# nmichlo/mtg-vision

Hardware: AMD Instinct MI355X
Metric: cards/sec end-to-end (detect+embed+top-1 over 100k bank), 640x640 (higher is better)
Workload: dtype f32 (products as 3 x f16 MFMA on hi/lo-split operands, f32 accumulate)

## Files before the change

### include/mtgv.h

```cpp
#ifndef MTGV_H
#define MTGV_H

#include <stddef.h>
#include <stdint.h>

#ifdef __cplusplus
extern "C" {
#endif

#if defined(__GNUC__)
#define MTGV_API __attribute__((visibility("default")))
#else
#define MTGV_API
#endif

MTGV_API const char* mtgv_last_error(void);
MTGV_API int mtgv_version(void);
MTGV_API int mtgv_device_count(void);

#define MTGV_PREC_F32 0
#define MTGV_PREC_F16X3 1
MTGV_API int mtgv_set_gemm_precision(int32_t prec);
MTGV_API int mtgv_get_gemm_precision(int32_t* prec);

// ... 133 lines not shown
MTGV_API int mtgv_op_linear_ex(const float* a_dev, const float* w_dev, const float* bias_dev, const float* res_dev, float* out_dev,
                               int32_t m, int32_t n, int32_t k, int32_t act, int32_t hw, const float* a_scale_dev,
                               const float* a_shift_dev, float* grn_part_dev, void* stream);
MTGV_API int mtgv_op_conv2d(const float* x_dev, const float* w_dev, const float* bias_dev, float* out_dev, int32_t n, int32_t h,
                            int32_t w, int32_t cin, int32_t cout, int32_t kh, int32_t kw, int32_t stride, int32_t pad,
                            int32_t act, void* stream);
MTGV_API int mtgv_op_layernorm(const float* x_dev, const float* w_dev, const float* b_dev, float* out_dev, int64_t rows,
                               int32_t c, float eps, void* stream);
MTGV_API int mtgv_op_dwconv7(const float* x_dev, const float* w49_dev, const float* bias_dev, float* out_dev, int32_t n,
                             int32_t h, int32_t w, int32_t c, void* stream);
MTGV_API int mtgv_op_block(const float* x_dev, float* out_dev, int32_t n, int32_t h, int32_t w, int32_t c, int32_t act,
                           const float* dw_w49, const float* dw_b, const float* ln_w, const float* ln_b, const float* w1,
                           const float* b1, const float* gamma, const float* beta, const float* w2, const float* b2,
                           float* ws_dev, void* stream);
MTGV_API int64_t mtgv_op_block_workspace_floats(int32_t n, int32_t h, int32_t w, int32_t c);
MTGV_API int mtgv_op_l2norm(const float* x_dev, float* out_dev, int64_t rows, int32_t d, void* stream);

#ifdef __cplusplus
}
#endif
#endif
```

### mtg-vision_amd/csrc/api.hip

```cpp
#include "mtgv.h"

#include <math.h>
#include <string.h>
#include <algorithm>
#include <mutex>

#include "encoder.h"
#include "match.h"
#include "rowops.h"
#include "gemm_sp.h"

namespace mtgv {
const char* last_error_cstr();
}

using namespace mtgv;

namespace {
std::recursive_mutex g_op_mu;
struct ScopedWeights {
  const float* w = nullptr;
  hipStream_t s;
  std::unique_lock<std::recursive_mutex> lk;
  ScopedWeights(const float* W, int n, int k, hipStream_t stream) : s(stream), lk(g_op_mu) {
// ... 305 lines not shown
    bw.dw_w49 = (float*)dw_w49, bw.dw_b = (float*)dw_b, bw.ln_w = (float*)ln_w, bw.ln_b = (float*)ln_b;
    bw.w1 = (float*)w1, bw.b1 = (float*)b1, bw.gamma = (float*)gamma, bw.beta = (float*)beta;
    bw.w2 = (float*)w2, bw.b2 = (float*)b2;
    ScopedWeights reg1(w1, 4 * c, c, (hipStream_t)stream), reg2(w2, c, 4 * c, (hipStream_t)stream);
    const BlockWsSize z = block_ws_size(n, h, w, c);
    BlockWs ws;
    ws.t1 = ws_dev;
    ws.t2 = ws.t1 + z.t;
    ws.hid = ws.t2 + z.t;
    ws.part = ws.hid + z.hid;
    ws.scale = ws.part + z.part;
    ws.bfold = ws.scale + z.scale;
    run_block(x_dev, out_dev, n, h, w, c, act, bw, ws, (hipStream_t)stream);
  });
}
MTGV_API int mtgv_op_l2norm(const float* x_dev, float* out_dev, int64_t rows, int32_t d, void* stream) {
  return guarded([&] {
    MTGV_CHECK(x_dev && out_dev, ERR_INVALID, "null argument");
    l2norm_rows_launch(x_dev, out_dev, rows, d, (hipStream_t)stream);
  });
}

}
```

### mtg-vision_amd/csrc/encoder.hip

```cpp
#include "encoder.h"
#include <stdlib.h>
#include "rowops.h"
#include "gemm_sp.h"
#include "mlp_fused.h"

#include <string.h>

namespace mtgv {

void DevBuf::alloc(size_t floats) {
  release();
  if (floats == 0) return;
  HIP_OK(hipMalloc((void**)&p, floats * sizeof(float)));
  n = floats;
}
void DevBuf::release() {
  if (p) (void)hipFree(p);
  p = nullptr;
  n = 0;
}

ParamStore::~ParamStore() {
  for (auto& kv : slots_)
    if (kv.second.dev) {
// ... 119 lines not shown
      fold_shift_into_bias_launch(bw.w2, bw.beta, bw.b2, ws.bfold, c, 4 * c, s);
      m.b2 = ws.bfold;
    }
    if (ln != nullptr && ln->out_sp8 != nullptr) m.out_ln = ln->out_sp8, m.ln_w = ln->w, m.ln_b = ln->b, m.ln_eps = ln->eps;
    mlp_fused_launch(m, s);
    return m.out_ln != nullptr;
  }

  GemmArgs g1 = linear_args(ws.t2, c, bw.w1, bw.b1, ws.hid, 4 * c, M, 4 * c, c, act);
  g1.a_fmt = fmt;
  g1.hw = hw;
  g1.grn_part = ws.part;
  const GrnLayout gl = gemm_grn_layout(g1);
  gemm_launch(g1, s);

  grn_finalize_launch(ws.part, gl, n, hw, 4 * c, bw.gamma, ws.scale, s);

  GemmArgs g2 = linear_args(ws.hid, 4 * c, bw.w2, bw.b2, out, c, M, c, 4 * c, ACT_NONE);
  g2.res = x;
  g2.ldr = c;
  g2.hw = hw;
  g2.a_scale = ws.scale;
  if (bw.b2_folded != nullptr) {
    g2.bias = bw.b2_folded;
  } else {
    fold_shift_into_bias_launch(bw.w2, bw.beta, bw.b2, ws.bfold, c, 4 * c, s);
    g2.bias = ws.bfold;
  }
  gemm_launch(g2, s);
  return false;
}

static std::string blk_key(int kind, int s, int j, const char* leaf) {
  char b[128];
  if (kind == MTGV_ENC_AE)
    snprintf(b, sizeof(b), "block%d.2.%d.%s", s, j, leaf);
  else
// ... 221 lines not shown
  MTGV_CHECK(x != nullptr && z_out != nullptr, ERR_INVALID, "null tensor");
  if (!prepared_) prepare();
  const int H = cfg_.image_h, W = cfg_.image_w;
  const float sc = cfg_.scale_io ? 2.0f : 1.0f, sf = cfg_.scale_io ? -1.0f : 0.0f;
  if (layout == MTGV_IN_NCHW_F32)
    nchw_to_nhwc_launch((const float*)x, x0_.p, n, 3, H, W, 3, sc, sf, s);
  else if (layout == MTGV_IN_NHWC_F32)
    f32hwc_scale_launch((const float*)x, x0_.p, (long)n * H * W, 3, 3, sc, sf, s);
  else if (layout == MTGV_IN_NHWC_U8)
    u8_to_f32_launch((const uint8_t*)x, x0_.p, (long)n * H * W, 3, 3, sc, sf, 0, s);
  else
    MTGV_CHECK(false, ERR_INVALID, "unknown input layout %d", layout);

  if (graph_mode_ != 0 && !capture_ && n <= graph_max_n_ && !gemm_profile_enabled()) {
    zbuf_.ensure((size_t)cfg_.max_batch * cfg_.z_size);
    const int gkey = n * 2 + gemm_precision();
    auto it = graphs_.find(gkey);
    if (it == graphs_.end()) {
      body(n, zbuf_.p, s);
      hipGraph_t graph = nullptr;
      hipGraphExec_t exec = nullptr;
      if (cap_stream_ == nullptr) HIP_OK(hipStreamCreateWithFlags(&cap_stream_, hipStreamNonBlocking));
      HIP_OK(hipStreamBeginCapture(cap_stream_, hipStreamCaptureModeThreadLocal));
      try {
        body(n, zbuf_.p, cap_stream_);
      } catch (...) {
        (void)hipStreamEndCapture(cap_stream_, &graph);
        if (graph) (void)hipGraphDestroy(graph);
        throw;
      }
      HIP_OK(hipStreamEndCapture(cap_stream_, &graph));
// ... 118 lines not shown
```

### mtg-vision_amd/csrc/gemm_f32.h

```cpp
#pragma once
#include "common.h"

namespace mtgv {

struct GemmArgs {
  const float* A = nullptr;
  int a_fmt = 0;
  const float* W = nullptr;
  const float* W_split = nullptr;
  const float* wscale = nullptr;
  float a_mul = 1.0f, a_unmul = 1.0f;
  float* Out = nullptr;
  int out_fmt = 0;
  const float* bias = nullptr;
  const float* res = nullptr;
  int res_fmt = 0;
  int M = 0, N = 0, K = 0;

  int H = 1, Wd = 1;
  int c_total = 0;
  int c_off = 0;
  int Cin = 0;
  int KH = 1, KW = 1, stride = 1, pad = 0;
  int stride_w = 0;
// ... 3 lines not shown
  int os = 1, oy = 0, ox = 0, OH2 = 1, OW2 = 1;
  int os_nq = 0;
  const float* W2 = nullptr;
  const float* bias2 = nullptr;
  float* Out2 = nullptr;
  int N2 = 0, ldo2 = 0, o_off2 = 0, out_fmt2 = 0, act2 = ACT_NONE;
  int ldr = 0;
  int act = ACT_NONE;

  float* grn_part = nullptr;
  int hw = 0;
  int segmax = 0;
  int grn_unit_rows = 0;
  const float* a_scale = nullptr;
  const float* a_shift = nullptr;

  int batch = 1;
  long strideA = 0, strideW = 0, strideO = 0;
  const int* m_count = nullptr;
  const float* crop_boxes = nullptr;
  int crop_rows = 0;
  float crop_scale = 0.f;
  int crop_w = 1;

  float* cand_s = nullptr;
  int* cand_i = nullptr;
  int topk = 0;
  const float* ln_w = nullptr;
  const float* ln_b = nullptr;
  float ln_eps = 0.f;
// ... 19 lines not shown
void gemm_profile_enable(bool on);
bool gemm_profile_enabled();
void gemm_profile_read(double* ms, double* flops, long* launches);
void gemm_profile_dump(const char* path);
double gemm_profile_bytes();
void gemm_profile_begin(const GemmArgs& a, hipStream_t s, int sp, double fill, double bytes);
void gemm_profile_end(hipStream_t s);

struct GrnLayout {
  int unit_rows = 0, segmax = 0;
  size_t floats = 0;
};
GrnLayout gemm_grn_layout(const GemmArgs& a);
size_t gemm_grn_part_floats_max(int M, int N, int hw);

void grn_finalize_launch(const float* part, const GrnLayout& l, int n_img, int hw, int N, const float* gamma, float* scale,
                         hipStream_t s);

}
```

### mtg-vision_amd/csrc/gemm_f32.hip

```cpp
#include "gemm_kernel.h"
#include "gemm_sp.h"

#include <stdlib.h>
#include <string.h>
#include <algorithm>
#include <map>
#include <mutex>
#include <string>
#include <vector>

namespace mtgv {

bool gemm_dispatch_f32(const GemmDev& g, const GemmPlan& pl, bool conv, bool apro, int grid, hipStream_t s) {
  return gemm_dispatch<0>(g, pl, conv, apro, grid, s);
}
bool gemm_dispatch_f16x3(const GemmDev& g, const GemmPlan& pl, bool conv, bool apro, int grid, hipStream_t s);


namespace {
struct GemmProf {
  bool on = false;
  std::vector<hipEvent_t> ev;
  size_t used = 0;
  double flops = 0;
// ... 34 lines not shown
double gemm_profile_bytes() { return g_prof.bytes; }

void gemm_profile_read(double* ms, double* flops, long* launches) {
  double total = 0;
  for (size_t i = 0; i + 1 < g_prof.used; i += 2) {
    HIP_OK(hipEventSynchronize(g_prof.ev[i + 1]));
    float t = 0.f;
    HIP_OK(hipEventElapsedTime(&t, g_prof.ev[i], g_prof.ev[i + 1]));
    total += t;
  }
  if (ms) *ms = total;
  if (flops) *flops = g_prof.flops;
  if (launches) *launches = g_prof.launches;
}

static void prof_begin(const GemmArgs& a, const GemmPlan& pl, hipStream_t s, int sp, double fill, double bytes_override = -1.0) {
  if (!g_prof.on) return;
  while (g_prof.ev.size() < g_prof.used + 2) {
    hipEvent_t e;
    HIP_OK(hipEventCreate(&e));
    g_prof.ev.push_back(e);
  }
  HIP_OK(hipEventRecord(g_prof.ev[g_prof.used], s));
  const double xfl = a.W2 != nullptr ? 2.0 * (double)a.M * a.N2 * a.N : 0.0;
  g_prof.flops += 2.0 * (double)a.M * a.N * a.K * a.batch + xfl;
  {
    const double a_el = is_conv(a) ? (double)(a.M / (a.OH * a.OW)) * a.H * a.Wd * a.Cin : (double)a.M * a.K;
    const double w_el = (double)a.N * a.K;
    const double o_el = a.topk > 0 ? (double)a.M * ceil_div(a.N, 64) * a.topk * 2
                                   : (a.W2 != nullptr ? (double)a.M * a.N2 + (double)a.N2 * a.N : (double)a.M * a.N);
    const double r_el = a.res != nullptr ? (double)a.M * a.N : 0.0;
    double by = 4.0 * ((a.strideA != 0 || a.batch == 1 ? a.batch : 1) * a_el + (a.strideW != 0 || a.batch == 1 ? a.batch : 1) * w_el +
                       a.batch * (o_el + r_el));
    if (bytes_override >= 0.0) by = bytes_override;
    g_prof.bytes += by;
    g_prof.recs.push_back({a.M, a.N, a.K, a.KH, a.stride, a.batch, a.act, a.a_scale != nullptr, a.grn_part != nullptr, a.topk,
                           pl.tm, pl.tn, pl.bk, sp, by, fill, xfl});
  }
  g_prof.launches += 1;
}
static void prof_end(hipStream_t s) {
  if (!g_prof.on) return;
  HIP_OK(hipEventRecord(g_prof.ev[g_prof.used + 1], s));
  g_prof.used += 2;
}

__global__ __launch_bounds__(256) void split_pack_kernel(const float* __restrict__ in, float* __restrict__ out, long n4) {
  const long i = (long)blockIdx.x * 256 + threadIdx.x;
  if (i >= n4) return;
// ... 210 lines not shown
  MTGV_CHECK((long)a.M * (long)(a.OH * a.OW > a.hw ? a.OH * a.OW : a.hw) < (1l << 40), ERR_INVALID, "gemm: M too large for fastdiv");
  const bool conv = is_conv(a);
  const bool apro = a.a_scale != nullptr;
  MTGV_CHECK(!(apro && conv), ERR_INVALID, "gemm: GRN prologue only on 1x1");
  MTGV_CHECK(!(apro && a.act != ACT_NONE), ERR_INVALID, "gemm: GRN prologue is only combined with a linear epilogue");
  MTGV_CHECK(a.a_shift == nullptr, ERR_INVALID, "gemm: fold the GRN shift into the bias (fold_shift_into_bias_launch)");
  if (!conv) MTGV_CHECK(a.OH == a.H && a.OW == a.Wd, ERR_INVALID, "gemm: 1x1 geometry mismatch");
  if (apro || a.grn_part) MTGV_CHECK(a.hw > 0 && a.M % a.hw == 0, ERR_INVALID, "gemm: hw=%d must divide M=%d", a.hw, a.M);
  const SpPlan sp = gemm_sp_plan(a);
  if (a.grn_part) {
    const GrnLayout l = grn_layout(a, sp, pl);
    a.segmax = l.segmax;
    a.grn_unit_rows = l.unit_rows;
  }
  if (sp.cfg >= 0) {
    prof_begin(a, pl, s, 1, g_prof.on ? gemm_sp_fill_bytes(a, sp) : 0.0);
    gemm_sp_launch(a, sp, s);
    prof_end(s);
    return;
  }

  MTGV_CHECK(a.os_nq == 0, ERR_INVALID, "gemm: the grouped scatter epilogue (os_nq) exists on the LDS-DMA kernel only");
  MTGV_CHECK(a.W2 == nullptr, ERR_INVALID, "gemm: the chained 1x1 exists on the LDS-DMA kernel only");
  GemmDev g;
  g.a = a;
  if (gemm_precision() == GEMM_PREC_F16X3 && g.a.W_split == nullptr && a.strideW == 0)
    g.a.W_split = split_for_launch(a.W, a.K, &g.a.wscale);
  if (gemm_precision() != GEMM_PREC_F16X3) g.a.W_split = nullptr, g.a.wscale = nullptr;
  g.d_ohw = make_fastdiv((uint32_t)(a.OH * a.OW));
  g.d_ow = make_fastdiv((uint32_t)a.OW);
  g.d_cin = make_fastdiv((uint32_t)a.Cin);
// ... 52 lines not shown
    }
    const float gval = sqrtf(sum);
    gx[n] = gval;
    local += gval;
  }
  red[tid] = local;
  __syncthreads();
  for (int st = 128; st > 0; st >>= 1) {
    if (tid < st) red[tid] += red[tid + st];
    __syncthreads();
  }
  const float denom = red[0] / (float)N + 1e-6f;
  for (int n = tid; n < N; n += 256) scale[(long)img * N + n] = gamma[n] * (gx[n] / denom) + 1.0f;
}

__global__ __launch_bounds__(256) void fold_shift_kernel(const float* __restrict__ W, const float* __restrict__ shift,
                                                        const float* __restrict__ bias, float* __restrict__ out, int N, int K) {
  const int lane = threadIdx.x & 63;
  const int n = blockIdx.x * 4 + (threadIdx.x >> 6);
  if (n >= N) return;
  float acc = 0.f;
  for (int k = lane; k < K; k += 64) acc += W[(long)n * K + k] * shift[k];
#pragma unroll
  for (int m = 32; m > 0; m >>= 1) acc += __shfl_xor(acc, m);
  if (lane == 0) out[n] = acc + (bias != nullptr ? bias[n] : 0.f);
}

void fold_shift_into_bias_launch(const float* W, const float* shift, const float* bias, float* out, int N, int K, hipStream_t s) {
  hipLaunchKernelGGL(fold_shift_kernel, dim3((N + 3) / 4), dim3(256), 0, s, W, shift, bias, out, N, K);
  HIP_OK(hipGetLastError());
}

void grn_finalize_launch(const float* part, const GrnLayout& l, int n_img, int hw, int N, const float* gamma, float* scale,
                         hipStream_t s) {
  const size_t lds = (size_t)(N + 256) * sizeof(float);
  MTGV_CHECK(lds <= 160 * 1024, ERR_INVALID, "grn_finalize: N=%d too large", N);
  hipLaunchKernelGGL(grn_finalize_kernel, dim3(n_img), dim3(256), lds, s, part, l.unit_rows, l.segmax, hw, N,
                     make_fastdiv((uint32_t)hw), make_fastdiv((uint32_t)l.unit_rows), gamma, scale);
  HIP_OK(hipGetLastError());
}

}
```

### mtg-vision_amd/csrc/gemm_sp.h

```cpp
#pragma once
#include "gemm_f32.h"

namespace mtgv {

void sp8_register(const float* W, size_t n_floats, int row_k);
void sp8_refresh(const float* W, size_t offset_floats, size_t n_floats, hipStream_t s);
void sp8_unregister(const float* W);
bool sp8_lookup(const float* W, int K, const char** sp8, const float** wscale);

struct SpPlan {
  int cfg = -1;
  int bm = 0, bn = 0;
  int unit_rows = 0;
  int tiles_m = 0, tiles_n = 0;
};

bool gemm_sp_active();
SpPlan gemm_sp_plan(const GemmArgs& a);
bool gemm_sp_takes_sp8(const float* W, int M, int N, int K, int lda, int c_off);
void gemm_sp_launch(const GemmArgs& a, const SpPlan& pl, hipStream_t s);
bool gemm_sp_chain_ok(const GemmArgs& a);
bool gemm_sp_topk_layout(const GemmArgs& a, int* slots, int* cols);
double gemm_sp_fill_bytes(const GemmArgs& a, const SpPlan& pl);
void gemm_sp_stamps_dump(const char* path);

void gemm_sp_topk_hi16_launch(const void* q_hi, const void* bank_hi, const float* wscale, int b, int N, int K, int kp, float* cand_s,
                              int* cand_i, int* slots, hipStream_t s);
int gemm_sp_topk_hi16_slots(int N);
int gemm_sp_topk_hi16_range_cols();

const char* sp_zero_page();

void sp8_pack_plain_launch(const float* in, void* out, long rows, int K, hipStream_t s);

}
```

### mtg-vision_amd/csrc/gemm_sp.hip

```cpp
#include "gemm_sp.h"

#include <stdlib.h>
#include <map>
#include <mutex>
#include <vector>

#include "gemm_sp_kernel.h"

namespace mtgv {

__global__ __launch_bounds__(256) void sp8_pack_rows_kernel(const float* __restrict__ in, sp_h8* __restrict__ out,
                                                           float* __restrict__ wscale, long rows, int K) {
  const int lane = threadIdx.x & 63;
  const long row = (long)blockIdx.x * 4 + (threadIdx.x >> 6);
  if (row >= rows) return;
  const float* x = in + row * K;
  float mx = 0.f;
  for (int k = lane; k < K; k += 64) mx = fmaxf(mx, fabsf(x[k]));
#pragma unroll
  for (int m = 32; m > 0; m >>= 1) mx = fmaxf(mx, __shfl_xor(mx, m));
  int e = 0;
  if (mx > 0.f && mx < INFINITY) {
    int ex;
    (void)frexpf(mx, &ex);
// ... 266 lines not shown
bool stamps_on() {
  static const bool on = [] { const char* e = getenv("MTGV_SP_STAMPS"); return e != nullptr && atoi(e) != 0; }();
  return on;
}
}

bool gemm_sp_topk_layout(const GemmArgs& a, int* slots, int* cols) {
  const SpPlan pl = gemm_sp_plan(a);
  if (pl.cfg < 0) return false;
  const SpCfg& k = kCfg[pl.cfg];
  *slots = pl.tiles_n * k.wn;
  *cols = 32 * k.tn;
  return true;
}

double gemm_sp_fill_bytes(const GemmArgs& a, const SpPlan& pl) {
  const SpCfg& k = kCfg[pl.cfg];
  const double tiles = (double)pl.tiles_m * pl.tiles_n;
  const double b_tile = (double)k.bn() * a.K * 4.0;
  double a_tile = (double)k.bm() * a.K * 4.0;
  if (a.a_fmt == 1 && is_conv(a) && window_conv_fits(a, pl)) a_tile = (double)window_bytes(k, a.Wd) * (a.Cin / k.kps());
  if (a.a_scale != nullptr) a_tile += (double)(a.K / 32) * 1024.0;
  return tiles * (a_tile + b_tile);
}

void gemm_sp_stamps_dump(const char* path) {
  if (g_stamps.empty()) return;
  HIP_OK(hipDeviceSynchronize());
  FILE* f = fopen(path, "wb");
  MTGV_CHECK(f != nullptr, ERR_RUNTIME, "cannot open %s", path);
  std::vector<long> host;
  for (const StampRec& r : g_stamps) {
    const int hdr[8] = {r.M, r.N, r.K, r.cfg, r.amode, r.act, r.tiles, 0};
    fwrite(hdr, sizeof(int), 8, f);
    host.resize((size_t)r.tiles * 8);
    HIP_OK(hipMemcpy(host.data(), r.buf, host.size() * sizeof(long), hipMemcpyDeviceToHost));
    fwrite(host.data(), sizeof(long), host.size(), f);
// ... 76 lines not shown
    g.W2 = w28, g.wscale2 = w2s, g.bias2 = a.bias2, g.Out2 = a.Out2, g.ldo2 = a.ldo2, g.o_off2 = a.o_off2, g.out_fmt2 = a.out_fmt2;
    g.act2 = a.act2, g.N2 = a.N2;
  }
  g.nq = a.os_nq;
  g.d_nq = make_fastdiv((uint32_t)(a.os_nq > 0 ? a.os_nq : 1)), g.d_os = make_fastdiv((uint32_t)(a.os > 0 ? a.os : 1));
  if (a.os_nq > 0)
    MTGV_CHECK(g.remap && a.os_nq % 8 == 0 && a.N == a.os * a.os * a.os_nq && a.oy == 0 && a.ox == 0 && a.res == nullptr &&
                   a.grn_part == nullptr,
               ERR_INVALID, "gemm_sp: os_nq=%d does not describe a %dx%d scatter of N=%d columns", a.os_nq, a.os, a.os, a.N);
  int amode = a.a_fmt == 1 ? (is_conv(a) ? 2 : 0) : 1;
  if (amode == 2 && window_conv_fits(a, pl)) amode = 5;
  if (amode == 1 && g.a_mul == 1.0f && ((uintptr_t)g.A & 15) == 0) {
    if (g.a_scale == nullptr) amode = 4;
    else if (((uintptr_t)g.a_scale & 15) == 0 && (kCfg[pl.cfg].bm() - 1) / g.hw + 2 <= 8) amode = 3;
  }
  if (stamps_on() && gemm_profile_enabled()) {
    const int tiles = pl.tiles_m * pl.tiles_n;
    long* buf = nullptr;
    HIP_OK(hipMalloc(&buf, (size_t)tiles * 8 * sizeof(long)));
    HIP_OK(hipMemsetAsync(buf, 0, (size_t)tiles * 8 * sizeof(long), s));
    g.stamps = buf;
    g_stamps.push_back({a.M, a.N, a.K, pl.cfg, amode, a.act, tiles, buf});
  }
  switch (pl.cfg) {
    case 0: gemm_sp_launch_cfg0(g, amode, s); break;
    case 1: gemm_sp_launch_cfg1(g, amode, s); break;
    case 2: gemm_sp_launch_cfg2(g, amode, s); break;
    case 3: gemm_sp_launch_cfg3(g, amode, s); break;
    case 4: gemm_sp_launch_cfg4(g, amode, s); break;
    case 5: gemm_sp_launch_cfg5(g, amode, s); break;
// ... 8 lines not shown
```

### mtg-vision_amd/csrc/gemm_sp_inst.h

```cpp
#pragma once
#include "gemm_sp_kernel.h"

namespace mtgv {

namespace {
#ifndef SP_KS_VALUE
#define SP_KS_VALUE 2
#endif
constexpr int SP_KS = SP_KS_VALUE;
#ifndef SP_NST
#define SP_NST 2
#endif

template <int AMODE, int ACT, int EPI, int NST = SP_NST>
void sp_launch_nst(const SpDev& g, hipStream_t s) {
  constexpr int BM = 32 * SP_TM * SP_WM, BN = 32 * SP_TN * SP_WN;
  constexpr size_t ring = (size_t)NST * ((AMODE == 5 ? BN : BM + BN) * 64 * SP_KS + (AMODE == 3 ? 1024 : 0));
  size_t lds = ring;
  constexpr size_t chain_lds = (size_t)SP_WM * SP_WN * 4096 * (1 + SP_TN) + (size_t)SP_TN * 96 * 128;
  if (AMODE == 5) {
    constexpr int RB = 64 * SP_KS, RPP = 1024 / RB;
    const size_t win = (size_t)((BM + 2 * g.Wd + 2 + RPP - 1) / RPP * RPP) * RB;
    const size_t stage = (size_t)SP_WM * SP_WN * 32 * 128 * SP_TN;
    lds = win + ring > stage ? win + ring : stage;
  }
  if (EPI == 32 && lds < chain_lds) lds = chain_lds;
  static bool attr_done_dev[MTGV_MAX_DEVICES] = {};
  bool& attr_done = attr_done_dev[current_device()];
  auto kern = gemm_sp_kernel<SP_WM, SP_WN, SP_TM, SP_TN, SP_KS, NST, AMODE, ACT, EPI>;
  if (!attr_done) {
    HIP_OK(hipFuncSetAttribute((const void*)kern, hipFuncAttributeMaxDynamicSharedMemorySize, (AMODE == 5 || EPI == 32) ? 160 * 1024 : (int)lds));
    attr_done = true;
  }
  hipLaunchKernelGGL(kern, dim3((unsigned)(g.tiles_m * g.tiles_n)), dim3(64 * SP_WM * SP_WN), lds, s, g);
}

template <int AMODE, int ACT, int EPI>
void sp_launch_one(const SpDev& g, hipStream_t s) {
  if constexpr (AMODE == 5 && SP_NST == 2) {
    constexpr int BM = 32 * SP_TM * SP_WM, BN = 32 * SP_TN * SP_WN, RB = 64 * SP_KS, RPP = 1024 / RB;
    const size_t win = (size_t)((BM + 2 * g.Wd + 2 + RPP - 1) / RPP * RPP) * RB;
    if ((long)g.tiles_m * g.tiles_n <= 512 && win + (size_t)4 * BN * RB <= 80 * 1024) {
      sp_launch_nst<AMODE, ACT, EPI, 4>(g, s);
      return;
    }
  }
// ... 54 lines not shown
      case ACT_MISH: sp_pick<0, ACT_MISH, 8>(g, epi, s); break;
      case ACT_GELU: sp_pick<0, ACT_GELU, 8>(g, epi, s); break;
      case ACT_SILU: sp_pick<0, ACT_SILU, 1, 5>(g, epi, s); break;
      default: sp_pick<0, -1>(g, epi, s); break;
    }
  } else if (amode == 1) {
#if SP_NST == 2
    if (g.act == ACT_NONE) sp_pick<1, ACT_NONE>(g, epi, s);
    else sp_pick<1, -1>(g, epi, s);
#else
    MTGV_CHECK(false, ERR_RUNTIME, "gemm_sp: the register A path has no deep-ring instance");
#endif
  } else if (amode == 3) {
    if (g.act == ACT_NONE) sp_pick<3, ACT_NONE, 2>(g, epi, s);
    else sp_pick<3, -1>(g, epi, s);
  } else if (amode == 4) {
    if (g.act == ACT_NONE) sp_pick<4, ACT_NONE, 0, 2>(g, epi, s);
    else sp_pick<4, -1>(g, epi, s);
  } else if (amode == 5) {
#if SP_NST == 2
    switch (g.act) {
#if SP_WN == 1 && SP_TM == 1
      case ACT_SILU: sp_pick<5, ACT_SILU, 1, 5, 32>(g, epi, s); break;
#else
      case ACT_SILU: sp_pick<5, ACT_SILU, 1, 5>(g, epi, s); break;
#endif
      default: sp_pick<5, -1>(g, epi, s); break;
    }
#else
    MTGV_CHECK(false, ERR_RUNTIME, "gemm_sp: the window conv has no deep-ring instance");
// ... 17 lines not shown
```

### mtg-vision_amd/csrc/gemm_sp_kernel.h

```cpp
#pragma once
#include <type_traits>

#include "act.h"
#include "gemm_f32.h"
#include "sp8.h"

namespace mtgv {

typedef float spf16 __attribute__((ext_vector_type(16)));

__device__ __forceinline__ spf16 sp_mfma(sp_h8 b, sp_h8 a, spf16 c) {
  return __builtin_amdgcn_mfma_f32_32x32x16_f16(b, a, c, 0, 0, 0);
}

struct SpDev {
  float* cand_s = nullptr;
  int* cand_i = nullptr;
  int topk = 0;
  long* stamps = nullptr;
  const char* A = nullptr;
  long a_rowb = 0;
  long a_offb = 0;
  const char* W = nullptr;
  const float* wscale = nullptr;
  const float* bias = nullptr;
  const void* res = nullptr;
  long ldr = 0;
  int res_fmt = 0;
  float* Out = nullptr;
  long ldo = 0;
  int o_off = 0;
  int out_fmt = 0;
  int M = 0, N = 0, K = 0;
  float* grn_part = nullptr;
  int hw = 1, segmax = 0;
  FastDiv d_hw;
  const float* a_scale = nullptr;
  float a_mul = 1.0f, a_unmul = 1.0f;
  const char* zero = nullptr;
  int off32 = 0;
  int tiles_m = 0, tiles_n = 0;
  int act = 0;
  int H = 1, Wd = 1, Cin = 0, KW = 1, stride = 1, pad = 0, OH = 1, OW = 1;
  FastDiv d_ohw, d_ow, d_cin, d_kw;
  int remap = 0, os = 1, oy = 0, ox = 0, OH2 = 1, OW2 = 1;
  int nq = 0;
  FastDiv d_nq, d_os;
  const char* W2 = nullptr;
  const float* wscale2 = nullptr;
  const float* bias2 = nullptr;
  float* Out2 = nullptr;
  long ldo2 = 0;
// ... 1 lines not shown
};

typedef const __attribute__((address_space(1))) void* sp_gptr;
typedef __attribute__((address_space(3))) void* sp_lptr;

template <int WM, int WN, int TM, int TN, int KS, int NST, int AMODE, int ACT, int EPI>
__global__ __launch_bounds__(64 * WM * WN, (WM * WN == 8 ? 4 : 2)) void gemm_sp_kernel(const SpDev g) {
#pragma clang fp contract(off)
  constexpr int NW = WM * WN, NT = 64 * NW, BM = 32 * TM * WM, BN = 32 * TN * WN;
  constexpr bool GEN = EPI < 0;
  static_assert(TM <= 2, "the epilogue names its slabs");
  static_assert(NST >= 2 && NST <= 4 && (AMODE != 1 || NST == 2), "ring depth; the register A path is two-deep");
  constexpr int RB = 64 * KS, RPP = 1024 / RB, SPR = RB / 16;
  constexpr bool AWIN = AMODE == 5;
  constexpr bool ADMA = AMODE != 1 && !AWIN;
  constexpr bool AF32 = AMODE == 3 || AMODE == 4;
  constexpr bool HI16 = AMODE == 6;
  constexpr int EB = HI16 ? 2 : 4;
  static_assert(!HI16 || (KS == 2 && EPI == 16), "fp16 rows: 128-byte stage rows, top-k epilogue");
  constexpr int SA = AWIN ? 0 : BM * RB, SB = BN * RB, SSC = AMODE == 3 ? 1024 : 0, STG = SA + SB + SSC;
  static_assert(AMODE != 3 || KS == 2, "the scale image is one DMA piece: 8 images x 32 k");
  constexpr int PA = ADMA ? BM / RPP : 0, PB = BN / RPP, NP = PA + PB;
  constexpr int PPW = (NP + NW - 1) / NW;
  constexpr int CPS = BM * 2 * KS;
  constexpr int CPT = AMODE == 1 ? CPS / NT : 1;
  static_assert(AMODE != 1 || CPS % NT == 0, "A chunks must divide over the threads");
  extern __shared__ __attribute__((aligned(1024))) char smem[];

  const int tid = threadIdx.x, lane = tid & 63;
  const int wave = __builtin_amdgcn_readfirstlane(tid >> 6);
  const int wm = wave / WN, wn = wave % WN;
// ... 46 lines not shown
        const uint32_t ow = rem - oh * (uint32_t)g.OW;
        cih0[u] = (int)oh * g.stride - g.pad;
        ciw0[u] = (int)ow * g.stride - g.pad;
        csrc[u] = g.A + (((long)img * g.H + cih0[u]) * g.Wd + ciw0[u]) * g.a_rowb + g.a_offb + slot * 16;
        src[u] = g.A + (long)img * g.H * g.Wd * g.a_rowb + g.a_offb + (slot & 1) * 16;
      } else {
        src[u] = g.A + (long)m * g.a_rowb + g.a_offb + slot * 16;
      }
    } else {
      int n = n0 + row;
      n = n < g.N ? n : g.N - 1;
      src[u] = g.W + (long)n * wrowb + slot * 16;
    }
    tailz[u] = ktail && ((nk - 1) * 2 * KS + (slot >> 1)) >= kchunks;
  }
  const int img0 = AMODE == 3 ? (int)fdiv((uint32_t)m0, g.d_hw) : 0;
  const char* sc_src = nullptr;
  bool sc_tailz = false;
  if constexpr (AMODE == 3) {
    const int img_last = (int)fdiv((uint32_t)(g.M - 1), g.d_hw);
    const int im = img0 + (lane >> 3) < img_last ? img0 + (lane >> 3) : img_last;
    sc_src = reinterpret_cast<const char*>(g.a_scale + (long)im * g.K) + (lane & 7) * 16;
    sc_tailz = ktail && ((nk - 1) * 2 * KS + ((lane & 7) >> 1)) >= kchunks;
  }
  const int win_px = AWIN ? ((BM + 2 * g.Wd + 2 + RPP - 1) / RPP * RPP) : 0;
  char* const ring = smem + (AWIN ? win_px * RB : 0);
  auto issue_piece = [&](int u, int t, int buf) {
    const int p = wave + NW * u;
    const char* s;
    if (AMODE == 2 && p < PA && conv_fast) {
      const uint32_t k0 = (uint32_t)t * (16u * KS);
// ... 147 lines not shown
  const int swr = KS == 2 ? (r >> 1) & 7 : (r >> 2) & 3;
  unsigned a_off[TM], b_off[TN];
#pragma unroll
  for (int i = 0; i < TM; ++i) a_off[i] = (unsigned)((wm * TM * 32 + i * 32 + r) * RB);
#pragma unroll
  for (int j = 0; j < TN; ++j) b_off[j] = (unsigned)(SA + (wn * TN * 32 + j * 32 + r) * RB);
  unsigned sc_off[TM];
#pragma unroll
  for (int i = 0; i < TM; ++i) {
    sc_off[i] = 0;
    if constexpr (AMODE == 3) {
      int m = m0 + wm * TM * 32 + i * 32 + r;
      m = m < g.M ? m : g.M - 1;
      sc_off[i] = (unsigned)(SA + SB + ((int)fdiv((uint32_t)m, g.d_hw) - img0) * 128 + h * 32);
    }
  }

  const int nw0 = n0 + wn * TN * 32;
  const int mw0 = m0 + wm * TM * 32;
  const int slot = lane & 7, lrow = lane >> 3;
  sp_f4 wsc[TN], bsv[TN];
  bool col_ok[TN];
  auto load_colvecs = [&]() {
#pragma unroll
  for (int j = 0; j < TN; ++j) {
    const int n = nw0 + j * 32 + slot * 4;
    col_ok[j] = n < g.N;
    sp_f4 w1 = {1.f, 1.f, 1.f, 1.f}, b0 = {0.f, 0.f, 0.f, 0.f};
    if (n + 4 <= g.N) {
      if (g.wscale != nullptr) w1 = *reinterpret_cast<const sp_f4*>(g.wscale + n);
      if (g.bias != nullptr) b0 = *reinterpret_cast<const sp_f4*>(g.bias + n);
    } else if (GEN && n < g.N) {
#pragma unroll
      for (int e = 0; e < 4; ++e)
        if (n + e < g.N) {
          if (g.wscale != nullptr) w1[e] = g.wscale[n + e];
          if (g.bias != nullptr) b0[e] = g.bias[n + e];
        }
    }
    wsc[j] = w1 * g.a_unmul;
    bsv[j] = b0;
  }
  };
  load_colvecs();

  const bool wave_active = m0 + wm * TM * 32 < g.M;

  int my_pieces = 0;
#pragma unroll
  for (int u = 0; u < PPW; ++u) my_pieces += (NP % NW == 0 || wave + NW * u < NP) ? 1 : 0;
  if (AMODE == 3 && wave == NP % NW) my_pieces += 1;
  constexpr int AHEAD = NST - 2;
  auto wait_stage = [&](bool tail) {
    if (AHEAD == 0 || tail) {
      asm volatile("s_waitcnt vmcnt(0) lgkmcnt(0)" ::: "memory");
    } else if (my_pieces == PPW) {
      asm volatile("s_waitcnt vmcnt(%0) lgkmcnt(0)" ::"n"(PPW * AHEAD) : "memory");
    } else if (my_pieces == PPW + 1) {
      asm volatile("s_waitcnt vmcnt(%0) lgkmcnt(0)" ::"n"((PPW + 1) * AHEAD) : "memory");
// ... 90 lines not shown
          sp_h8 ah[TM], bh[TN];
  #pragma unroll
          for (int i = 0; i < TM; ++i) ah[i] = *reinterpret_cast<const sp_h8*>(sb + a_off[i] + so);
  #pragma unroll
          for (int j = 0; j < TN; ++j) bh[j] = *reinterpret_cast<const sp_h8*>(sb + b_off[j] + so);
  #pragma unroll
          for (int j = 0; j < TN; ++j)
  #pragma unroll
            for (int i = 0; i < TM; ++i) acc[i][j] = sp_mfma(bh[j], ah[i], acc[i][j]);
        }
      }
      if constexpr (AF32 && KS == 2 && !HI16) {
        __builtin_amdgcn_sched_barrier(0);
        if (wave_active) {
          const char* const sb = ring + buf * STG;
          sp_f4 xa[2][TM][2], xs[2][TM][2];
          sp_h8 bh[2][TN], bl[2][TN];
  #pragma unroll
          for (int ks = 0; ks < 2; ++ks) {
            const unsigned shi = (unsigned)(((ks * 4 + h * 2 + 0) ^ swr) << 4);
            const unsigned slo = (unsigned)(((ks * 4 + h * 2 + 1) ^ swr) << 4);
  #pragma unroll
            for (int i = 0; i < TM; ++i) {
              xa[ks][i][0] = *reinterpret_cast<const sp_f4*>(sb + a_off[i] + shi);
              xa[ks][i][1] = *reinterpret_cast<const sp_f4*>(sb + a_off[i] + slo);
              if constexpr (AMODE == 3) {
                xs[ks][i][0] = *reinterpret_cast<const sp_f4*>(sb + sc_off[i] + ks * 64);
                xs[ks][i][1] = *reinterpret_cast<const sp_f4*>(sb + sc_off[i] + ks * 64 + 16);
              }
            }
  #pragma unroll
            for (int j = 0; j < TN; ++j) {
              bh[ks][j] = *reinterpret_cast<const sp_h8*>(sb + b_off[j] + shi);
              bl[ks][j] = *reinterpret_cast<const sp_h8*>(sb + b_off[j] + slo);
            }
          }
          if constexpr (AMODE == 3) {
  #pragma unroll
            for (int ks = 0; ks < 2; ++ks)
  #pragma unroll
              for (int i = 0; i < TM; ++i) xa[ks][i][0] = xa[ks][i][0] * xs[ks][i][0], xa[ks][i][1] = xa[ks][i][1] * xs[ks][i][1];
          }
          sp_h8 ah[2][TM], al[2][TM];
  #pragma unroll
          for (int i = 0; i < TM; ++i) sp8_split8_mix(xa[0][i][0], xa[0][i][1], ah[0][i], al[0][i]);
  #pragma unroll
          for (int ks = 0; ks < 2; ++ks) {
            if (ks == 0) {
  #pragma unroll
              for (int i = 0; i < TM; ++i) sp8_split8_mix(xa[1][i][0], xa[1][i][1], ah[1][i], al[1][i]);
            }
  #pragma unroll
            for (int j = 0; j < TN; ++j)
  #pragma unroll
              for (int i = 0; i < TM; ++i) acc[i][j] = sp_mfma(bl[ks][j], ah[ks][i], acc[i][j]);
  #pragma unroll
            for (int j = 0; j < TN; ++j)
  #pragma unroll
              for (int i = 0; i < TM; ++i) acc[i][j] = sp_mfma(bh[ks][j], al[ks][i], acc[i][j]);
  #pragma unroll
            for (int j = 0; j < TN; ++j)
  #pragma unroll
              for (int i = 0; i < TM; ++i) acc[i][j] = sp_mfma(bh[ks][j], ah[ks][i], acc[i][j]);
          }
          constexpr int CV = (AMODE == 3 ? 8 : 0) + 16;
          __builtin_amdgcn_sched_group_barrier(0x100, 2 * (TM * (AMODE == 3 ? 4 : 2) + 2 * TN), 0);
          __builtin_amdgcn_sched_group_barrier(0x002, CV * TM, 0);
  #pragma unroll
          for (int q = 0; q < 3 * TM * TN; ++q) {
            __builtin_amdgcn_sched_group_barrier(0x008, 1, 0);
            __builtin_amdgcn_sched_group_barrier(0x002, (CV * TM + 3 * TM * TN - 1) / (3 * TM * TN), 0);
          }
        }
      } else if (wave_active && !HI16) {
        const char* const sb = ring + buf * STG;
  #pragma unroll
        for (int ks = 0; ks < KS; ++ks) {
          const unsigned shi = (unsigned)(((ks * 4 + h * 2 + 0) ^ swr) << 4);
          const unsigned slo = (unsigned)(((ks * 4 + h * 2 + 1) ^ swr) << 4);
          sp_h8 ah[TM], al[TM], bh[TN], bl[TN];
  #pragma unroll
// ... 405 lines not shown
```

### mtg-vision_amd/mtgv/native.py

```python

from __future__ import annotations

import ctypes as C
import os

import torch

_HERE = os.path.dirname(os.path.abspath(__file__))
LIB_PATH = os.environ.get("MTGV_LIB_PATH", os.path.join(_HERE, "libmtgv.so"))

c_i32, c_i64, c_f32, c_vp = C.c_int32, C.c_int64, C.c_float, C.c_void_p
c_fp = C.POINTER(C.c_float)


class EncoderCfg(C.Structure):
    _fields_ = [
        ("kind", c_i32),
        ("image_h", c_i32),
        ("image_w", c_i32),
        ("in_chans", c_i32),
        ("z_size", c_i32),
        ("depths", c_i32 * 4),
        ("dims", c_i32 * 4),
        ("head_type", c_i32),
# ... 74 lines not shown
    "mtgv_jpeg_decode": (C.c_int, [c_vp, c_vp, c_vp, c_vp, c_i32, c_vp, c_vp, c_vp, c_vp, c_vp]),
    "mtgv_jpeg_encode_bound": (C.c_int, [c_i32, c_i32, c_i32, C.POINTER(c_i64)]),
    "mtgv_jpeg_encode_header": (C.c_int, [c_i32, c_i32, c_i32, c_i32, c_vp, c_i64, C.POINTER(c_i64)]),
    "mtgv_jpeg_encoder_create": (C.c_int, [c_i32, c_i64, C.POINTER(c_vp)]),
    "mtgv_jpeg_encoder_destroy": (None, [c_vp]),
    "mtgv_jpeg_encode": (C.c_int, [c_vp, c_vp, c_i32, c_i32, c_i32, c_i32, c_i32, c_vp, c_i64, c_vp, c_vp]),
    "mtgv_op_linear": (C.c_int, [c_vp, c_vp, c_vp, c_vp, c_vp, c_i32, c_i32, c_i32, c_i32, c_vp]),
    "mtgv_op_linear_ex_part_floats": (c_i64, [c_i32, c_i32, c_i32, c_i32, c_i32]),
    "mtgv_op_last_grn_layout": (C.c_int, [c_vp, c_vp]),
    "mtgv_op_linear_ex": (C.c_int, [c_vp, c_vp, c_vp, c_vp, c_vp, c_i32, c_i32, c_i32, c_i32, c_i32, c_vp, c_vp, c_vp, c_vp]),
    "mtgv_op_conv2d": (C.c_int, [c_vp, c_vp, c_vp, c_vp] + [c_i32] * 10 + [c_vp]),
    "mtgv_op_layernorm": (C.c_int, [c_vp, c_vp, c_vp, c_vp, c_i64, c_i32, c_f32, c_vp]),
    "mtgv_op_dwconv7": (C.c_int, [c_vp, c_vp, c_vp, c_vp, c_i32, c_i32, c_i32, c_i32, c_vp]),
    "mtgv_op_block": (C.c_int, [c_vp, c_vp, c_i32, c_i32, c_i32, c_i32, c_i32] + [c_vp] * 10 + [c_vp, c_vp]),
    "mtgv_op_block_workspace_floats": (c_i64, [c_i32, c_i32, c_i32, c_i32]),
    "mtgv_op_l2norm": (C.c_int, [c_vp, c_vp, c_i64, c_i32, c_vp]),
}

_lib = None


def lib():
    global _lib
    if _lib is None:
        if not os.path.exists(LIB_PATH):
            raise RuntimeError(
                f"{LIB_PATH} is missing: build it with `python mtg-vision_amd/build.py` "
                "(mtgv has no CPU or eager fallback for the recognition path)"
            )
        L = C.CDLL(LIB_PATH)
# ... 49 lines not shown
```

Baseline: 32730.

## Derive GRN scale inside the second MLP GEMM prologue instead of a finalize kernel

Adds a new A-mode (7) to the split-precision GEMM kernel. In this mode each workgroup reduces the GRN partial sums for the images its tile touches, computes the per-channel scale table in LDS, and applies it while loading A. The separate grn_finalize kernel launch between the two MLP GEMMs is skipped whenever the inline path qualifies. The trade-off is that every tile redundantly re-reads and reduces the partials and uses extra LDS, which may reduce occupancy. An env var toggle, launch counters and a graph key bit are added.

```diff
diff --git a/include/mtgv.h b/include/mtgv.h
--- a/include/mtgv.h
+++ b/include/mtgv.h
@@ -171,6 +171,7 @@
                            const float* b1, const float* gamma, const float* beta, const float* w2, const float* b2,
                            float* ws_dev, void* stream);
 MTGV_API int64_t mtgv_op_block_workspace_floats(int32_t n, int32_t h, int32_t w, int32_t c);
+MTGV_API int mtgv_grn_launch_counts(int64_t* finalize, int64_t* inline_derived);
 MTGV_API int mtgv_op_l2norm(const float* x_dev, float* out_dev, int64_t rows, int32_t d, void* stream);
 
 #ifdef __cplusplus
diff --git a/mtg-vision_amd/csrc/api.hip b/mtg-vision_amd/csrc/api.hip
--- a/mtg-vision_amd/csrc/api.hip
+++ b/mtg-vision_amd/csrc/api.hip
@@ -343,6 +343,14 @@
     run_block(x_dev, out_dev, n, h, w, c, act, bw, ws, (hipStream_t)stream);
   });
 }
+MTGV_API int mtgv_grn_launch_counts(int64_t* finalize, int64_t* inline_derived) {
+  return guarded([&] {
+    MTGV_CHECK(finalize && inline_derived, ERR_INVALID, "null argument");
+    long f = 0, d = 0;
+    gemm_grn_launch_counts(&f, &d);
+    *finalize = f, *inline_derived = d;
+  });
+}
 MTGV_API int mtgv_op_l2norm(const float* x_dev, float* out_dev, int64_t rows, int32_t d, void* stream) {
   return guarded([&] {
     MTGV_CHECK(x_dev && out_dev, ERR_INVALID, "null argument");
diff --git a/mtg-vision_amd/csrc/encoder.hip b/mtg-vision_amd/csrc/encoder.hip
--- a/mtg-vision_amd/csrc/encoder.hip
+++ b/mtg-vision_amd/csrc/encoder.hip
@@ -157,13 +157,13 @@
   const GrnLayout gl = gemm_grn_layout(g1);
   gemm_launch(g1, s);
 
-  grn_finalize_launch(ws.part, gl, n, hw, 4 * c, bw.gamma, ws.scale, s);
-
   GemmArgs g2 = linear_args(ws.hid, 4 * c, bw.w2, bw.b2, out, c, M, c, 4 * c, ACT_NONE);
   g2.res = x;
   g2.ldr = c;
   g2.hw = hw;
   g2.a_scale = ws.scale;
+  g2.grn_src = ws.part, g2.grn_src_unit_rows = gl.unit_rows, g2.grn_src_segmax = gl.segmax, g2.grn_gamma = bw.gamma;
+  if (!gemm_derives_grn(g2)) grn_finalize_launch(ws.part, gl, n, hw, 4 * c, bw.gamma, ws.scale, s);
   if (bw.b2_folded != nullptr) {
     g2.bias = bw.b2_folded;
   } else {
@@ -415,7 +415,7 @@
 
   if (graph_mode_ != 0 && !capture_ && n <= graph_max_n_ && !gemm_profile_enabled()) {
     zbuf_.ensure((size_t)cfg_.max_batch * cfg_.z_size);
-    const int gkey = n * 2 + gemm_precision();
+    const int gkey = (n * 2 + gemm_precision()) * 2 + (gemm_grn_inline_enabled() ? 1 : 0);
     auto it = graphs_.find(gkey);
     if (it == graphs_.end()) {
       body(n, zbuf_.p, s);
diff --git a/mtg-vision_amd/csrc/gemm_f32.h b/mtg-vision_amd/csrc/gemm_f32.h
--- a/mtg-vision_amd/csrc/gemm_f32.h
+++ b/mtg-vision_amd/csrc/gemm_f32.h
@@ -41,6 +41,9 @@
   int grn_unit_rows = 0;
   const float* a_scale = nullptr;
   const float* a_shift = nullptr;
+  const float* grn_src = nullptr;
+  int grn_src_unit_rows = 0, grn_src_segmax = 0;
+  const float* grn_gamma = nullptr;
 
   int batch = 1;
   long strideA = 0, strideW = 0, strideO = 0;
@@ -90,6 +93,10 @@
 GrnLayout gemm_grn_layout(const GemmArgs& a);
 size_t gemm_grn_part_floats_max(int M, int N, int hw);
 
+bool gemm_derives_grn(const GemmArgs& a);
+bool gemm_grn_inline_enabled();
+void gemm_grn_launch_counts(long* finalize, long* inline_derived);
+
 void grn_finalize_launch(const float* part, const GrnLayout& l, int n_img, int hw, int N, const float* gamma, float* scale,
                          hipStream_t s);
 
diff --git a/mtg-vision_amd/csrc/gemm_f32.hip b/mtg-vision_amd/csrc/gemm_f32.hip
--- a/mtg-vision_amd/csrc/gemm_f32.hip
+++ b/mtg-vision_amd/csrc/gemm_f32.hip
@@ -4,6 +4,7 @@
 #include <stdlib.h>
 #include <string.h>
 #include <algorithm>
+#include <atomic>
 #include <map>
 #include <mutex>
 #include <string>
@@ -72,7 +73,8 @@
   if (launches) *launches = g_prof.launches;
 }
 
-static void prof_begin(const GemmArgs& a, const GemmPlan& pl, hipStream_t s, int sp, double fill, double bytes_override = -1.0) {
+static void prof_begin(const GemmArgs& a, const GemmPlan& pl, hipStream_t s, int sp, double fill, double bytes_override = -1.0,
+                       double bytes_extra = 0.0) {
   if (!g_prof.on) return;
   while (g_prof.ev.size() < g_prof.used + 2) {
     hipEvent_t e;
@@ -91,6 +93,7 @@
     double by = 4.0 * ((a.strideA != 0 || a.batch == 1 ? a.batch : 1) * a_el + (a.strideW != 0 || a.batch == 1 ? a.batch : 1) * w_el +
                        a.batch * (o_el + r_el));
     if (bytes_override >= 0.0) by = bytes_override;
+    by += bytes_extra;
     g_prof.bytes += by;
     g_prof.recs.push_back({a.M, a.N, a.K, a.KH, a.stride, a.batch, a.act, a.a_scale != nullptr, a.grn_part != nullptr, a.topk,
                            pl.tm, pl.tn, pl.bk, sp, by, fill, xfl});
@@ -331,7 +334,9 @@
     a.grn_unit_rows = l.unit_rows;
   }
   if (sp.cfg >= 0) {
-    prof_begin(a, pl, s, 1, g_prof.on ? gemm_sp_fill_bytes(a, sp) : 0.0);
+    const bool derives = g_prof.on && gemm_sp_derives_grn(a, sp);
+    prof_begin(a, pl, s, 1, g_prof.on ? gemm_sp_fill_bytes(a, sp) : 0.0, -1.0,
+               derives ? (double)ceil_div(a.M, a.grn_src_unit_rows) * a.grn_src_segmax * a.K * 4.0 : 0.0);
     gemm_sp_launch(a, sp, s);
     prof_end(s);
     return;
@@ -414,6 +419,13 @@
   for (int n = tid; n < N; n += 256) scale[(long)img * N + n] = gamma[n] * (gx[n] / denom) + 1.0f;
 }
 
+static std::atomic<long> g_grn_finalize_launches{0};
+void gemm_grn_inline_count(long* n);
+void gemm_grn_launch_counts(long* finalize, long* inline_derived) {
+  *finalize = g_grn_finalize_launches.load();
+  gemm_grn_inline_count(inline_derived);
+}
+
 __global__ __launch_bounds__(256) void fold_shift_kernel(const float* __restrict__ W, const float* __restrict__ shift,
                                                         const float* __restrict__ bias, float* __restrict__ out, int N, int K) {
   const int lane = threadIdx.x & 63;
@@ -433,6 +445,7 @@
 
 void grn_finalize_launch(const float* part, const GrnLayout& l, int n_img, int hw, int N, const float* gamma, float* scale,
                          hipStream_t s) {
+  g_grn_finalize_launches += 1;
   const size_t lds = (size_t)(N + 256) * sizeof(float);
   MTGV_CHECK(lds <= 160 * 1024, ERR_INVALID, "grn_finalize: N=%d too large", N);
   hipLaunchKernelGGL(grn_finalize_kernel, dim3(n_img), dim3(256), lds, s, part, l.unit_rows, l.segmax, hw, N,
diff --git a/mtg-vision_amd/csrc/gemm_sp.h b/mtg-vision_amd/csrc/gemm_sp.h
--- a/mtg-vision_amd/csrc/gemm_sp.h
+++ b/mtg-vision_amd/csrc/gemm_sp.h
@@ -21,6 +21,7 @@
 void gemm_sp_launch(const GemmArgs& a, const SpPlan& pl, hipStream_t s);
 bool gemm_sp_chain_ok(const GemmArgs& a);
 bool gemm_sp_topk_layout(const GemmArgs& a, int* slots, int* cols);
+bool gemm_sp_derives_grn(const GemmArgs& a, const SpPlan& pl);
 double gemm_sp_fill_bytes(const GemmArgs& a, const SpPlan& pl);
 void gemm_sp_stamps_dump(const char* path);
 
diff --git a/mtg-vision_amd/csrc/gemm_sp.hip b/mtg-vision_amd/csrc/gemm_sp.hip
--- a/mtg-vision_amd/csrc/gemm_sp.hip
+++ b/mtg-vision_amd/csrc/gemm_sp.hip
@@ -1,6 +1,7 @@
 #include "gemm_sp.h"
 
 #include <stdlib.h>
+#include <atomic>
 #include <map>
 #include <mutex>
 #include <vector>
@@ -304,13 +305,47 @@
   return true;
 }
 
+namespace {
+std::atomic<long> g_grn_inline_launches{0};
+int grn_units_per_image(const GemmArgs& a) {
+  const int u = a.grn_src_unit_rows;
+  return (a.hw + u - 1) / u + (a.hw % u != 0 ? 1 : 0);
+}
+#ifndef MTGV_GRN_INLINE_MAX_TILE_BYTES
+#define MTGV_GRN_INLINE_MAX_TILE_BYTES (80 * 1024)
+#endif
+}
+
+bool gemm_grn_inline_enabled() {
+  const char* const e = getenv("MTGV_GRN_INLINE");
+  return e == nullptr || atoi(e) != 0;
+}
+
+bool gemm_sp_derives_grn(const GemmArgs& a, const SpPlan& pl) {
+  if (pl.cfg < 0 || a.grn_src == nullptr || a.grn_gamma == nullptr || a.grn_src_unit_rows <= 0 || a.grn_src_segmax <= 0) return false;
+  if (!gemm_grn_inline_enabled()) return false;
+  if (a.a_scale == nullptr || a.a_fmt == 1 || is_conv(a) || a.a_mul != 1.0f || ((uintptr_t)a.A & 15) != 0 || ((uintptr_t)a.a_scale & 15) != 0 ||
+      a.act != ACT_NONE || a.topk > 0 || a.hw <= 0)
+    return false;
+  const SpCfg& k = kCfg[pl.cfg];
+  const int nimg = (k.bm() - 1) / a.hw + 2;
+  if (nimg > 8 || k.wm * k.wn != 4 || k.ks != 2 || a.K % 32 != 0) return false;
+  const size_t ring = (size_t)2 * (k.bm() + k.bn()) * k.rb(), table = (size_t)nimg * a.K * 4;
+  if (ring + table > 80 * 1024) return false;
+  return (size_t)nimg * grn_units_per_image(a) * a.K * 4 <= (size_t)MTGV_GRN_INLINE_MAX_TILE_BYTES;
+}
+bool gemm_derives_grn(const GemmArgs& a) { return gemm_sp_derives_grn(a, gemm_sp_plan(a)); }
+
+void gemm_grn_inline_count(long* n) { *n = g_grn_inline_launches.load(); }
+
 double gemm_sp_fill_bytes(const GemmArgs& a, const SpPlan& pl) {
   const SpCfg& k = kCfg[pl.cfg];
   const double tiles = (double)pl.tiles_m * pl.tiles_n;
   const double b_tile = (double)k.bn() * a.K * 4.0;
   double a_tile = (double)k.bm() * a.K * 4.0;
   if (a.a_fmt == 1 && is_conv(a) && window_conv_fits(a, pl)) a_tile = (double)window_bytes(k, a.Wd) * (a.Cin / k.kps());
-  if (a.a_scale != nullptr) a_tile += (double)(a.K / 32) * 1024.0;
+  if (gemm_sp_derives_grn(a, pl)) a_tile += (double)((k.bm() - 1) / a.hw + 2) * grn_units_per_image(a) * a.K * 4.0;
+  else if (a.a_scale != nullptr) a_tile += (double)(a.K / 32) * 1024.0;
   return tiles * (a_tile + b_tile);
 }
 
@@ -417,6 +452,14 @@
     if (g.a_scale == nullptr) amode = 4;
     else if (((uintptr_t)g.a_scale & 15) == 0 && (kCfg[pl.cfg].bm() - 1) / g.hw + 2 <= 8) amode = 3;
   }
+  if (amode == 3 && gemm_sp_derives_grn(a, pl)) {
+    amode = 7;
+    g.a_scale = nullptr;
+    g.grn_src = a.grn_src, g.gamma = a.grn_gamma;
+    g.src_unit_rows = a.grn_src_unit_rows, g.src_segmax = a.grn_src_segmax;
+    g.d_src_unit = make_fastdiv((uint32_t)a.grn_src_unit_rows);
+    g_grn_inline_launches += 1;
+  }
   if (stamps_on() && gemm_profile_enabled()) {
     const int tiles = pl.tiles_m * pl.tiles_n;
     long* buf = nullptr;
diff --git a/mtg-vision_amd/csrc/gemm_sp_inst.h b/mtg-vision_amd/csrc/gemm_sp_inst.h
--- a/mtg-vision_amd/csrc/gemm_sp_inst.h
+++ b/mtg-vision_amd/csrc/gemm_sp_inst.h
@@ -25,11 +25,12 @@
     lds = win + ring > stage ? win + ring : stage;
   }
   if (EPI == 32 && lds < chain_lds) lds = chain_lds;
+  if (AMODE == 7) lds += (size_t)((BM - 1) / g.hw + 2) * g.K * 4;
   static bool attr_done_dev[MTGV_MAX_DEVICES] = {};
   bool& attr_done = attr_done_dev[current_device()];
   auto kern = gemm_sp_kernel<SP_WM, SP_WN, SP_TM, SP_TN, SP_KS, NST, AMODE, ACT, EPI>;
   if (!attr_done) {
-    HIP_OK(hipFuncSetAttribute((const void*)kern, hipFuncAttributeMaxDynamicSharedMemorySize, (AMODE == 5 || EPI == 32) ? 160 * 1024 : (int)lds));
+    HIP_OK(hipFuncSetAttribute((const void*)kern, hipFuncAttributeMaxDynamicSharedMemorySize, (AMODE == 5 || EPI == 32) ? 160 * 1024 : (AMODE == 7 ? 80 * 1024 : (int)lds)));
     attr_done = true;
   }
   hipLaunchKernelGGL(kern, dim3((unsigned)(g.tiles_m * g.tiles_n)), dim3(64 * SP_WM * SP_WN), lds, s, g);
@@ -114,6 +115,13 @@
   } else if (amode == 3) {
     if (g.act == ACT_NONE) sp_pick<3, ACT_NONE, 2>(g, epi, s);
     else sp_pick<3, -1>(g, epi, s);
+  } else if (amode == 7) {
+#if SP_WM * SP_WN == 4 && SP_NST == 2
+    MTGV_CHECK(g.act == ACT_NONE, ERR_RUNTIME, "gemm_sp: the GRN-deriving A mode has linear epilogues only");
+    sp_pick<7, ACT_NONE, 2>(g, epi, s);
+#else
+    MTGV_CHECK(false, ERR_RUNTIME, "gemm_sp: configuration %d cannot derive GRN multipliers (256 threads, two-deep ring)", SP_CFG_ID);
+#endif
   } else if (amode == 4) {
     if (g.act == ACT_NONE) sp_pick<4, ACT_NONE, 0, 2>(g, epi, s);
     else sp_pick<4, -1>(g, epi, s);
diff --git a/mtg-vision_amd/csrc/gemm_sp_kernel.h b/mtg-vision_amd/csrc/gemm_sp_kernel.h
--- a/mtg-vision_amd/csrc/gemm_sp_kernel.h
+++ b/mtg-vision_amd/csrc/gemm_sp_kernel.h
@@ -36,6 +36,10 @@
   int hw = 1, segmax = 0;
   FastDiv d_hw;
   const float* a_scale = nullptr;
+  const float* grn_src = nullptr;
+  const float* gamma = nullptr;
+  int src_unit_rows = 1, src_segmax = 0;
+  FastDiv d_src_unit;
   float a_mul = 1.0f, a_unmul = 1.0f;
   const char* zero = nullptr;
   int off32 = 0;
@@ -67,7 +71,10 @@
   constexpr int RB = 64 * KS, RPP = 1024 / RB, SPR = RB / 16;
   constexpr bool AWIN = AMODE == 5;
   constexpr bool ADMA = AMODE != 1 && !AWIN;
-  constexpr bool AF32 = AMODE == 3 || AMODE == 4;
+  constexpr bool AF32 = AMODE == 3 || AMODE == 4 || AMODE == 7;
+  constexpr bool AGRN = AMODE == 7;
+  constexpr bool ASC = AMODE == 3 || AGRN;
+  static_assert(!AGRN || (NT == 256 && NST == 2 && KS == 2), "the GRN prologue keeps grn_finalize_kernel's 256-slot sum; ring slot 1 is its scratch");
   constexpr bool HI16 = AMODE == 6;
   constexpr int EB = HI16 ? 2 : 4;
   static_assert(!HI16 || (KS == 2 && EPI == 16), "fp16 rows: 128-byte stage rows, top-k epilogue");
@@ -144,7 +151,7 @@
     }
     tailz[u] = ktail && ((nk - 1) * 2 * KS + (slot >> 1)) >= kchunks;
   }
-  const int img0 = AMODE == 3 ? (int)fdiv((uint32_t)m0, g.d_hw) : 0;
+  const int img0 = ASC ? (int)fdiv((uint32_t)m0, g.d_hw) : 0;
   const char* sc_src = nullptr;
   bool sc_tailz = false;
   if constexpr (AMODE == 3) {
@@ -322,6 +329,11 @@
       m = m < g.M ? m : g.M - 1;
       sc_off[i] = (unsigned)(SA + SB + ((int)fdiv((uint32_t)m, g.d_hw) - img0) * 128 + h * 32);
     }
+    if constexpr (AGRN) {
+      int m = m0 + wm * TM * 32 + i * 32 + r;
+      m = m < g.M ? m : g.M - 1;
+      sc_off[i] = (unsigned)(NST * STG + (((int)fdiv((uint32_t)m, g.d_hw) - img0) * g.K + h * 8) * 4);
+    }
   }
 
   const int nw0 = n0 + wn * TN * 32;
@@ -351,6 +363,59 @@
   }
   };
   load_colvecs();
+
+  if constexpr (AGRN) {
+    float* const tab = reinterpret_cast<float*>(smem + NST * STG);
+    float* const red = reinterpret_cast<float*>(smem + STG);
+    const int m_hi = m0 + BM - 1 < g.M ? m0 + BM - 1 : g.M - 1;
+    const int ni = (int)fdiv((uint32_t)m_hi, g.d_hw) - img0 + 1;
+    constexpr int KJ = 3, UG = 4;
+    for (int ii = 0; ii < ni; ++ii) {
+      const int img = img0 + ii;
+      const int t_first = (int)fdiv((uint32_t)(img * g.hw), g.d_src_unit);
+      const int t_last = (int)fdiv((uint32_t)((img + 1) * g.hw - 1), g.d_src_unit);
+      float local = 0.f;
+      for (int kb = tid; kb < g.K; kb += 256 * KJ) {
+        float sum[KJ];
+#pragma unroll
+        for (int j = 0; j < KJ; ++j) sum[j] = 0.f;
+        for (int t0 = t_first; t0 <= t_last; t0 += UG) {
+          float v[UG][KJ];
+#pragma unroll
+          for (int u = 0; u < UG; ++u) {
+            const int t = t0 + u <= t_last ? t0 + u : t_last;
+            const int seg = img - (int)fdiv((uint32_t)(t * g.src_unit_rows), g.d_hw);
+            const float* const row = g.grn_src + ((long)t * g.src_segmax + seg) * g.K;
+#pragma unroll
+            for (int j = 0; j < KJ; ++j) v[u][j] = (t0 + u <= t_last && kb + 256 * j < g.K) ? row[kb + 256 * j] : 0.f;
+          }
+#pragma unroll
+          for (int u = 0; u < UG; ++u)
+#pragma unroll
+            for (int j = 0; j < KJ; ++j) sum[j] += v[u][j];
+        }
+#pragma unroll
+        for (int j = 0; j < KJ; ++j)
+          if (kb + 256 * j < g.K) {
+            const float gval = sqrtf(sum[j]);
+            tab[ii * g.K + kb + 256 * j] = gval;
+            local += gval;
+          }
+      }
+      red[ii * 256 + tid] = local;
+    }
+    asm volatile("s_waitcnt lgkmcnt(0)" ::: "memory");
+    __builtin_amdgcn_s_barrier();
+    for (int ii = 0; ii < ni; ++ii) {
+      const float* const rr = red + ii * 256 + lane;
+      float c = (rr[0] + rr[128]) + (rr[64] + rr[192]);
+#pragma unroll
+      for (int st = 32; st > 0; st >>= 1) c += __shfl_down(c, st);
+      const float tot = __builtin_bit_cast(float, __builtin_amdgcn_readfirstlane(__builtin_bit_cast(int, c)));
+      const float denom = tot / (float)g.K + 1e-6f;
+      for (int k = tid; k < g.K; k += 256) tab[ii * g.K + k] = __builtin_fmaf(g.gamma[k], tab[ii * g.K + k] / denom, 1.0f);
+    }
+  }
 
   const bool wave_active = m0 + wm * TM * 32 < g.M;
 
@@ -471,6 +536,7 @@
         __builtin_amdgcn_sched_barrier(0);
         if (wave_active) {
           const char* const sb = ring + buf * STG;
+          const char* const scb = AGRN ? smem + t * (KPS * 4) : sb;
           sp_f4 xa[2][TM][2], xs[2][TM][2];
           sp_h8 bh[2][TN], bl[2][TN];
   #pragma unroll
@@ -481,9 +547,9 @@
             for (int i = 0; i < TM; ++i) {
               xa[ks][i][0] = *reinterpret_cast<const sp_f4*>(sb + a_off[i] + shi);
               xa[ks][i][1] = *reinterpret_cast<const sp_f4*>(sb + a_off[i] + slo);
-              if constexpr (AMODE == 3) {
-                xs[ks][i][0] = *reinterpret_cast<const sp_f4*>(sb + sc_off[i] + ks * 64);
-                xs[ks][i][1] = *reinterpret_cast<const sp_f4*>(sb + sc_off[i] + ks * 64 + 16);
+              if constexpr (ASC) {
+                xs[ks][i][0] = *reinterpret_cast<const sp_f4*>(scb + sc_off[i] + ks * 64);
+                xs[ks][i][1] = *reinterpret_cast<const sp_f4*>(scb + sc_off[i] + ks * 64 + 16);
               }
             }
   #pragma unroll
@@ -492,7 +558,7 @@
               bl[ks][j] = *reinterpret_cast<const sp_h8*>(sb + b_off[j] + slo);
             }
           }
-          if constexpr (AMODE == 3) {
+          if constexpr (ASC) {
   #pragma unroll
             for (int ks = 0; ks < 2; ++ks)
   #pragma unroll
@@ -520,8 +586,8 @@
   #pragma unroll
               for (int i = 0; i < TM; ++i) acc[i][j] = sp_mfma(bh[ks][j], ah[ks][i], acc[i][j]);
           }
-          constexpr int CV = (AMODE == 3 ? 8 : 0) + 16;
-          __builtin_amdgcn_sched_group_barrier(0x100, 2 * (TM * (AMODE == 3 ? 4 : 2) + 2 * TN), 0);
+          constexpr int CV = (ASC ? 8 : 0) + 16;
+          __builtin_amdgcn_sched_group_barrier(0x100, 2 * (TM * (ASC ? 4 : 2) + 2 * TN), 0);
           __builtin_amdgcn_sched_group_barrier(0x002, CV * TM, 0);
   #pragma unroll
           for (int q = 0; q < 3 * TM * TN; ++q) {
diff --git a/mtg-vision_amd/mtgv/native.py b/mtg-vision_amd/mtgv/native.py
--- a/mtg-vision_amd/mtgv/native.py
+++ b/mtg-vision_amd/mtgv/native.py
@@ -112,6 +112,7 @@
     "mtgv_op_dwconv7": (C.c_int, [c_vp, c_vp, c_vp, c_vp, c_i32, c_i32, c_i32, c_i32, c_vp]),
     "mtgv_op_block": (C.c_int, [c_vp, c_vp, c_i32, c_i32, c_i32, c_i32, c_i32] + [c_vp] * 10 + [c_vp, c_vp]),
     "mtgv_op_block_workspace_floats": (c_i64, [c_i32, c_i32, c_i32, c_i32]),
+    "mtgv_grn_launch_counts": (C.c_int, [c_vp, c_vp]),
     "mtgv_op_l2norm": (C.c_int, [c_vp, c_vp, c_i64, c_i32, c_vp]),
 }
 
```

Measured after the change: 32630, median of 2. No clear change (-0.3%).
